# MechaCritter/Python-Visual-Similarity

Hardware: AMD Instinct MI355X
Metric: images/sec encoded + top-k retrieved, VLAD K256 RootSIFT (higher is better)
Workload: dtype f32

## Files before the change

### include/pvsim.h

```cpp
#ifndef PVSIM_H
#define PVSIM_H

#include <stddef.h>
#include <stdint.h>

#ifdef __cplusplus
extern "C" {
#endif

#define PVS_VERSION 103

typedef enum {
  PVS_OK = 0,
  PVS_ERR_INVALID = 1,
  PVS_ERR_NO_DEVICE = 2,
  PVS_ERR_OOM = 3,
  PVS_ERR_UNSUPPORTED = 4,
  PVS_ERR_DIM = 5,
  PVS_ERR_CAPACITY = 6
} pvs_status;

typedef enum {
  PVS_DESC_F32 = 0,
  PVS_DESC_F32_ROOTSIFT = 1,
  PVS_DESC_U8_ROOTSIFT = 2
} pvs_desc_kind;

typedef enum {
  PVS_OPT_ASSIGN_PREFILTER = 0,
  PVS_OPT_VLAD_PATH = 1,
  PVS_OPT_TOPK_SELECT_ONLY = 2,
  PVS_OPT_AGG_VARIANT = 3,
  PVS_OPT_FISHER_SCALE = 4,
  PVS_OPT_TRAIN_BATCH_CHUNKS = 5,
  PVS_OPT_UPDATE_WINDOW_ROWS = 6,
  PVS_OPT_SQ8_PATH = 7,
  PVS_OPT_COUNT_ = 8
} pvs_option;

typedef struct pvs_ctx pvs_ctx;
typedef struct pvs_codebook pvs_codebook;
typedef struct pvs_gmm pvs_gmm;
typedef struct pvs_pca pvs_pca;
typedef struct pvs_comm pvs_comm;

typedef struct {
  double power_norm_weight;
  double norm_order;
  double epsilon;
} pvs_norm_params;

int pvs_version(void);
const char* pvs_last_error(void);
int pvs_device_count(int* count);
int pvs_init(int device_id, void* stream, pvs_ctx** out);
int pvs_destroy(pvs_ctx* ctx);
int pvs_sync(pvs_ctx* ctx);
void* pvs_stream(pvs_ctx* ctx);
int pvs_device_name(pvs_ctx* ctx, char* buf, size_t buflen);
int pvs_set_option(pvs_ctx* ctx, int option, int value);
// ... 292 lines not shown
```

### include/pvsim_diag.h

```cpp
#ifndef PVSIM_DIAG_H
#define PVSIM_DIAG_H

#include "pvsim.h"

#ifdef __cplusplus
extern "C" {
#endif

int pvs_fused_profile(pvs_ctx* ctx, int enable, int64_t* out16);

#ifdef __cplusplus
}
#endif
#endif
```

### python-visual-similarity_amd/csrc/api.hip

```cpp
#include <algorithm>
#include <cmath>
#include <limits>
#include <memory>

#include "panel_plan.hpp"

namespace pvs {

static thread_local char g_err[512] = "";

void set_error(const char* fmt, ...) {
  va_list ap;
  va_start(ap, fmt);
  vsnprintf(g_err, sizeof(g_err), fmt, ap);
  va_end(ap);
}

static_assert(WS_UPDATE + 1 == pvs_ctx::NWS, "one block per WsSlot");

int ws_reserve(pvs_ctx* ctx, WsSlot which, size_t bytes, void** out) {
  if (bytes == 0) bytes = 16;
  if (ctx->ws_bytes[which] < bytes) {
    if (ctx->ws[which]) {
      PVS_HIP(hipStreamSynchronize(ctx->stream));
// ... 142 lines not shown
  return PVS_OK;
}

PVS_EXPORT int pvs_destroy(pvs_ctx* ctx) {
  if (!ctx) return PVS_OK;
  hipSetDevice(ctx->device);
  hipStreamSynchronize(ctx->stream);
  drain_timers(ctx);
  for (hipEvent_t e : ctx->event_pool) (void)hipEventDestroy(e);
  ctx->event_pool.clear();
  for (auto& kv : ctx->block_cache) (void)hipFree(kv.second);
  ctx->block_cache.clear();
  if (ctx->h_stage) (void)hipHostFree(ctx->h_stage);
  for (int i = 0; i < pvs_ctx::DSIFT_RING; ++i) {
    if (ctx->dsift_h[i]) (void)hipHostFree(ctx->dsift_h[i]);
    if (ctx->dsift_ev[i]) (void)hipEventDestroy(ctx->dsift_ev[i]);
  }
  for (int i = 0; i < pvs_ctx::NWS; ++i)
    if (ctx->ws[i]) hipFree(ctx->ws[i]);
  for (auto& p : ctx->gemm_plan)
    if (p.d_tiles) hipFree(p.d_tiles);
  if (ctx->d_queue) hipFree(ctx->d_queue);
  if (ctx->d_fused_stamps) hipFree(ctx->d_fused_stamps);
  if (ctx->owns_stream) hipStreamDestroy(ctx->stream);
  delete ctx;
  return PVS_OK;
}

PVS_EXPORT int pvs_sync(pvs_ctx* ctx) {
  PVS_NEED(ctx, "ctx");
  PVS_HIP(hipStreamSynchronize(ctx->stream));
  return PVS_OK;
}

PVS_EXPORT void* pvs_stream(pvs_ctx* ctx) { return ctx ? static_cast<void*>(ctx->stream) : nullptr; }

PVS_EXPORT int pvs_device_name(pvs_ctx* ctx, char* buf, size_t buflen) {
  PVS_NEED(ctx, "ctx");
  PVS_NEED(buf, "buf");
  hipDeviceProp_t prop;
  PVS_HIP(hipGetDeviceProperties(&prop, ctx->device));
  snprintf(buf, buflen, "%s (%s, %d CUs)", prop.name, prop.gcnArchName, prop.multiProcessorCount);
  return PVS_OK;
}

PVS_EXPORT int pvs_set_option(pvs_ctx* ctx, int option, int value) {
// ... 978 lines not shown
  PVS_HIP(hipMemcpyAsync(h_indices, d_indices, (size_t)n_clusters * 8, hipMemcpyDeviceToHost, ctx->stream));
  PVS_HIP(hipStreamSynchronize(ctx->stream));
  return PVS_OK;
}

PVS_EXPORT int pvs_fused_profile(pvs_ctx* ctx, int enable, int64_t* out16) {
  PVS_NEED(ctx, "ctx");
  PVS_HIP(hipSetDevice(ctx->device));
  PVS_HIP(hipStreamSynchronize(ctx->stream));
  if (out16) {
    for (int i = 0; i < 16; ++i) out16[i] = 0;
    if (ctx->d_fused_stamps) PVS_HIP(hipMemcpy(out16, ctx->d_fused_stamps, 16 * 8, hipMemcpyDeviceToHost));
  }
  if (enable) {
    if (!ctx->d_fused_stamps) PVS_HIP(hipMalloc(reinterpret_cast<void**>(&ctx->d_fused_stamps), 16 * 8));
    PVS_HIP(hipMemset(ctx->d_fused_stamps, 0, 16 * 8));
  } else if (ctx->d_fused_stamps) {
    PVS_HIP(hipFree(ctx->d_fused_stamps));
    ctx->d_fused_stamps = nullptr;
  }
  return PVS_OK;
}

PVS_EXPORT int pvs_timers_enable(pvs_ctx* ctx, int on) {
  PVS_NEED(ctx, "ctx");
  PVS_TRY(drain_timers(ctx));
  ctx->timers_on = on != 0;
  return PVS_OK;
}
PVS_EXPORT int pvs_timers_reset(pvs_ctx* ctx) {
  PVS_NEED(ctx, "ctx");
  PVS_TRY(drain_timers(ctx));
  for (int i = 0; i < PVS_TIMER_SLOTS; ++i) {
    ctx->t_total[i] = 0;
    ctx->t_count[i] = 0;
  }
  return PVS_OK;
}
PVS_EXPORT int pvs_timers_read(pvs_ctx* ctx, int which, double* total_ms, int64_t* launches) {
  PVS_NEED(ctx, "ctx");
  if (which < 0 || which >= PVS_TIMER_SLOTS) PVS_FAIL(PVS_ERR_INVALID, "timer slot %d out of range", which);
  PVS_TRY(drain_timers(ctx));
  if (total_ms) *total_ms = ctx->t_total[which];
  if (launches) *launches = ctx->t_count[which];
  return PVS_OK;
}
// ... 1 lines not shown
```

### python-visual-similarity_amd/csrc/assign_prefilter.hpp

```cpp
#pragma once

#include "common.hpp"
#include "desc_load.hpp"

namespace pvs {

typedef _Float16 f16x8_t __attribute__((ext_vector_type(8)));
typedef _Float16 f16x4_t __attribute__((ext_vector_type(4)));

constexpr int ASSIGN_THREADS = 512;
constexpr int ASSIGN_ROWS = (ASSIGN_THREADS / 64) * 32;

struct Assign16Args {
  const void* X;
  int64_t total;
  int D, ld;
  const _Float16* C16;
  const float* cnorm;
  int K_pad, D_pad16;
  int c_shift;
  float cmax;
  const _Float16* cnk;
  int cn_e1, K;
  int32_t* labels;
  int64_t* amb_rows;
  unsigned long long* amb_count;
  int64_t cap;
  float2* rowstat;
  unsigned long long* stamps;
  int nprod;
  int shape16;
};

int launch_assign16x(pvs_ctx* ctx, const Assign16Args& p, int kind, size_t lds, int grid);

__device__ __forceinline__ void pf_fill_sqrt_table(uint32_t* lds_t) {
  if (threadIdx.x < 256) {
    const float sv = sqrtf((float)threadIdx.x);
    const _Float16 hi = (_Float16)sv, lo = (_Float16)(sv - (float)hi);
    lds_t[threadIdx.x] = (uint32_t)__builtin_bit_cast(unsigned short, hi) | ((uint32_t)__builtin_bit_cast(unsigned short, lo) << 16);
  }
}
__device__ __forceinline__ void pf_u8_fragment(const uint32_t* lds_t, const uint32_t* xw, f16x8_t* xh, f16x8_t* xl) {
  uint32_t hw[4], lw[4];
#pragma unroll
  for (int i = 0; i < 2; ++i)
#pragma unroll
    for (int pq = 0; pq < 2; ++pq) {
      const uint32_t w = xw[i];
      const uint32_t e0 = lds_t[(w >> (16 * pq)) & 0xffu], e1 = lds_t[(w >> (16 * pq + 8)) & 0xffu];
      hw[2 * i + pq] = __builtin_amdgcn_perm(e1, e0, 0x05040100u);
      lw[2 * i + pq] = __builtin_amdgcn_perm(e1, e0, 0x07060302u);
    }
  *xh = __builtin_bit_cast(f16x8_t, make_uint4(hw[0], hw[1], hw[2], hw[3]));
  *xl = __builtin_bit_cast(f16x8_t, make_uint4(lw[0], lw[1], lw[2], lw[3]));
}

// ... 26 lines not shown
```

### python-visual-similarity_amd/csrc/common.hpp

```cpp
#pragma once
#include <hip/hip_runtime.h>

#include <cmath>
#include <cstdarg>
#include <cstdint>
#include <cstdio>
#include <cstring>
#include <map>
#include <type_traits>
#include <vector>

#include "../../include/pvsim.h"
#include "../../include/pvsim_diag.h"
#include "workspace.hpp"

#define PVS_EXPORT extern "C" __attribute__((visibility("default")))

namespace pvs {

void set_error(const char* fmt, ...);

#define PVS_FAIL(code, ...)        \
  do {                             \
    ::pvs::set_error(__VA_ARGS__); \
// ... 27 lines not shown

struct TimerRec {
  hipEvent_t a, b;
  int slot;
};

}

struct pvs_ctx {
  int device = 0;
  hipStream_t stream = nullptr;
  bool owns_stream = false;
  int num_cu = 256;
  static constexpr int NWS = 18;
  void* ws[NWS] = {};
  size_t ws_bytes[NWS] = {};
  struct GemmPlanSlot {
    int key[4] = {-1, -1, -1, -1};
    int n_main = 0, n_tail = 0, splitk = 1;
    void* d_tiles = nullptr;
    size_t cap = 0;
  } gemm_plan[5];
  std::map<const void*, int> lds_attr;
  int opt[PVS_OPT_COUNT_] = {1, 0, 0, 0, 0, 0, 0, 0};
  unsigned int* d_queue = nullptr;
  unsigned long long* d_fused_stamps = nullptr;
  bool timers_on = false;
  std::vector<pvs::TimerRec> pending;
  std::vector<hipEvent_t> event_pool;
  std::multimap<size_t, void*> block_cache;
  std::map<void*, size_t> block_size;
  size_t block_cache_bytes = 0;
  void* h_stage = nullptr;
  size_t h_stage_bytes = 0;
  static constexpr int DSIFT_RING = 4;
  void* dsift_h[DSIFT_RING] = {};
  size_t dsift_h_bytes[DSIFT_RING] = {};
  hipEvent_t dsift_ev[DSIFT_RING] = {};
  int dsift_next = 0;
  double t_total[PVS_TIMER_SLOTS] = {0};
  int64_t t_count[PVS_TIMER_SLOTS] = {0};
};

struct pvs_codebook {
  int K = 0, D = 0;
  int K_pad = 0, D_pad = 0;
  float* d_cent = nullptr;
  float* d_cpad = nullptr;
  float* d_cnorm = nullptr;
// ... 169 lines not shown
```

### python-visual-similarity_amd/csrc/vlad.hip

```cpp
#include "assign_prefilter.hpp"

namespace pvs {

typedef float f32x16 __attribute__((ext_vector_type(16)));

struct AssignArgs {
  const void* X;
  int64_t total;
  int D, ld;
  const float* Cpad;
  const float* cnorm;
  int K_pad, D_pad;
  int32_t* labels;
  const int64_t* rows;
  const unsigned long long* nrows;
  int64_t rows_cap;
};

constexpr int ASSIGN_DCHUNK = 128;

template <int NT, int KIND, bool VEC>
__global__ __launch_bounds__(ASSIGN_THREADS, 2) void assign_kernel(AssignArgs a) {
  extern __shared__ __attribute__((aligned(16))) char smem[];
  constexpr int CB = 32 * NT;
// ... 2 lines not shown
  float* lds_c = reinterpret_cast<float*>(smem);
  float* lds_n = lds_c + CB * stride;

  const int lane = threadIdx.x & 63, wave = threadIdx.x >> 6;
  const int j = lane & 31, h = lane >> 5;
  const int ncb = a.K_pad / CB;
  const int nsc = (a.D_pad + ASSIGN_DCHUNK - 1) / ASSIGN_DCHUNK;
  const bool restage = (ncb * nsc) > 1;
  const int64_t n_items = a.rows ? (int64_t)a.nrows[blockIdx.x] : a.total;
  const int64_t nblocks = (n_items + ASSIGN_ROWS - 1) / ASSIGN_ROWS;
  const int64_t* const my_rows = a.rows ? a.rows + (int64_t)blockIdx.x * a.rows_cap : nullptr;

  auto stage = [&](int cb, int sc) {
    const int cw = min(ASSIGN_DCHUNK, a.D_pad - sc * ASSIGN_DCHUNK);
    const int c4n = cw >> 2;
    for (int idx = threadIdx.x; idx < CB * c4n; idx += ASSIGN_THREADS) {
      const int r = idx / c4n, c4 = idx - r * c4n;
      const float4 v = *reinterpret_cast<const float4*>(a.Cpad + (int64_t)(cb * CB + r) * a.D_pad +
                                                        sc * ASSIGN_DCHUNK + 4 * c4);
      *reinterpret_cast<float4*>(lds_c + r * stride + 4 * c4) = v;
    }
    for (int idx = threadIdx.x; idx < CB; idx += ASSIGN_THREADS) lds_n[idx] = a.cnorm[cb * CB + idx];
  };

  if (!restage) {
    stage(0, 0);
    __syncthreads();
  }

  for (int64_t blk = my_rows ? 0 : blockIdx.x; blk < nblocks; blk += my_rows ? 1 : gridDim.x) {
    const int64_t item = blk * ASSIGN_ROWS + wave * 32 + j;
    const bool rvalid = item < n_items;
    const int64_t row = (my_rows && rvalid) ? my_rows[item] : item;
    float best = INFINITY;
    int bidx = 0;

    for (int cb = 0; cb < ncb; ++cb) {
      f32x16 acc[NT];
#pragma unroll
      for (int t = 0; t < NT; ++t)
#pragma unroll
        for (int r = 0; r < 16; ++r) acc[t][r] = 0.f;

      for (int sc = 0; sc < nsc; ++sc) {
        if (restage) {
          __syncthreads();
// ... 485 lines not shown
  if (total <= 0) return PVS_OK;
  const bool rs = kind != PVS_DESC_F32;
  if (rs && cb->D > ASSIGN_DCHUNK)
    PVS_FAIL(PVS_ERR_UNSUPPORTED, "fused RootSIFT needs D <= %d (got %d)", ASSIGN_DCHUNK, cb->D);
  const int nt = assign_tiles_for(cb->K);
  if (cb->K_pad % (32 * nt) != 0) PVS_FAIL(PVS_ERR_INVALID, "codebook padding does not match the tile count");
  AssignArgs a{d_desc, total, cb->D, ld, cb->d_cpad, cb->d_cnorm, cb->K_pad, cb->D_pad, d_labels, nullptr, nullptr, 0};
  const int esz = kind == PVS_DESC_U8_ROOTSIFT ? 1 : 4;
  const bool vec = (cb->D % 4 == 0) && (ld % 4 == 0) && ((reinterpret_cast<uintptr_t>(d_desc) % (4 * esz)) == 0);
  const int cw = cb->D_pad < ASSIGN_DCHUNK ? cb->D_pad : ASSIGN_DCHUNK;
  const size_t lds = (size_t)(32 * nt) * (cw + 4) * 4 + (size_t)(32 * nt) * 4;
  const int64_t nblocks = (total + ASSIGN_ROWS - 1) / ASSIGN_ROWS;
  const int grid = (int)(nblocks < ctx->num_cu ? nblocks : ctx->num_cu);
  ScopedTimer tm(ctx, T_ASSIGN);
  const bool pre = cb->d_c16 != nullptr && total >= 4096 && ctx->opt[PVS_OPT_ASSIGN_PREFILTER] != 0;
  if (pre) {
    const int64_t cap = (nblocks + grid - 1) / grid * ASSIGN_ROWS;
    char* ws = nullptr;
    const bool stat = rowstat_out != nullptr && kind == PVS_DESC_U8_ROOTSIFT;
    WsLayout<> lay;
    const auto cnt_p = lay.add<unsigned long long>((size_t)grid);
    const auto rows_p = lay.add<int64_t>((size_t)grid * cap);
    const auto stat_p = lay.add<float2>(stat ? (size_t)total : 0);
    PVS_TRY(ws_reserve(ctx, WS_LISTS, lay.bytes(), &ws));
    unsigned long long* cnt = cnt_p(ws);
    int64_t* rows = rows_p(ws);
    float2* rowstat = stat ? stat_p(ws) : nullptr;
    if (stat) *rowstat_out = rowstat;
    Assign16Args p{d_desc, total, cb->D, ld, static_cast<const _Float16*>(cb->d_c16), cb->d_cnorm, cb->K_pad, cb->D_pad16,
                   cb->c16_shift, cb->cmax, static_cast<const _Float16*>(cb->d_cnk), cb->cn_e1, cb->K, d_labels, rows, cnt, cap, rowstat,
                   ctx->d_fused_stamps, ctx->opt[PVS_OPT_ASSIGN_PREFILTER] == 2 ? 2 : (ctx->opt[PVS_OPT_ASSIGN_PREFILTER] == 3 ? 1 : 3),
                   ctx->opt[PVS_OPT_ASSIGN_PREFILTER] == 4 ? 1 : 0};
    const size_t lds16 = (size_t)2 * cb->K_pad * (128 + 8) * 2 + (size_t)cb->K_pad * 4 + (size_t)cb->K_pad * 8 + 1024;
    PVS_TRY(launch_assign16(ctx, p, kind, cb->K_pad / 32, vec, lds16, grid));
    a.rows = rows;
    a.nrows = cnt;
    a.rows_cap = cap;
  }
  return dispatch_desc_kind(kind, [&](auto k) { return launch_assign_kind<decltype(k)::value>(ctx, a, nt, vec, lds, grid); });
}

struct AggArgs {
  const void* X;
  int D, ld;
  const int64_t* offsets;
  const int32_t* labels;
  const float* cent;
  int K;
  float power, eps;
  int norm_mode;
  float norm_p;
  float* out;
  float* inv_norm;
  const float2* rowstat;
};

constexpr int AGG_THREADS = 256;
constexpr int AGG_WAVES = AGG_THREADS / 64;
constexpr int AGG_CHUNK = 4096;

// ... 497 lines not shown
```

### python-visual-similarity_amd/csrc/vlad_fused.hip

```cpp
#include "common.hpp"
#include "desc_load.hpp"

namespace pvs {

typedef float f32x16 __attribute__((ext_vector_type(16)));
typedef _Float16 f16x8_t __attribute__((ext_vector_type(8)));
typedef _Float16 f16x4_t __attribute__((ext_vector_type(4)));

constexpr int FU_THREADS = 512;
constexpr int FU_R = 64;
constexpr int FU_XS = 132;
constexpr int FU_TS = 1056;
constexpr int FU_TILE = 8 * FU_TS;
constexpr int FU_UNUSABLE = 0x7fffffff;
constexpr int FU_KB = 4;

constexpr int FU_OFF_X32 = 0;
constexpr int FU_OFF_XH = FU_OFF_X32 + FU_R * FU_XS * 4;
constexpr int FU_OFF_XL = FU_OFF_XH + 2 * FU_TILE;
constexpr int FU_OFF_NX = FU_OFF_XL + 2 * FU_TILE;
constexpr int FU_OFF_XSH = FU_OFF_NX + 256;
constexpr int FU_OFF_CAND = FU_OFF_XSH + 256;
constexpr int FU_OFF_ENT = FU_OFF_CAND + 8 * FU_R * 8;
constexpr int FU_OFF_ENTV = FU_OFF_ENT + 2048;
constexpr int FU_OFF_ROWSQ = FU_OFF_ENTV + 4096;
constexpr int FU_OFF_MISC = FU_OFF_ROWSQ + 1024;
constexpr int FU_LDS = FU_OFF_MISC + 64;

struct FusedArgs {
  const void* X;
// ... 294 lines not shown
          if (wave == 0 && ne > 0) {
            int e = ebase;
            for (int w = 0; w < 8; ++w)
              if (cm & (1 << w)) {
                const int sidx = 31 - (__float_as_int(s_cand[w * FU_R + lane].x) & 31);
                s_ent[e++] = lane | (w << 8) | (((am >> w) & 1) << 12) | (sidx << 16);
              }
          }
          __syncthreads();
          for (int e0 = 0; e0 < E; e0 += 16) {
            const int e = e0 + 2 * wave + h;
            const bool elive = e < E;
            const int ent = elive ? s_ent[e] : 0;
            const int er = ent & 0xff, ew = (ent >> 8) & 7, eall = (ent >> 12) & 1, esi = (ent >> 16) & 31;
            const int k = 32 * ew + (eall ? j : esi);
            const bool active = elive && (eall || j == 0);
            const float* xr = x32 + er * FU_XS;
            const float* cr = a.cpad + (size_t)k * 128;
            float dot = 0.f;
#pragma unroll 2
            for (int b8 = 0; b8 < 128; b8 += 8) {
              const float4 xa = *reinterpret_cast<const float4*>(xr + b8), xb = *reinterpret_cast<const float4*>(xr + b8 + 4);
              const float4 ca = *reinterpret_cast<const float4*>(cr + b8), cb = *reinterpret_cast<const float4*>(cr + b8 + 4);
              dot = fmaf(ca.x, xa.x, dot); dot = fmaf(cb.x, xb.x, dot);
              dot = fmaf(ca.y, xa.y, dot); dot = fmaf(cb.y, xb.y, dot);
              dot = fmaf(ca.z, xa.z, dot); dot = fmaf(cb.z, xb.z, dot);
              dot = fmaf(ca.w, xa.w, dot); dot = fmaf(cb.w, xb.w, dot);
            }
            const float v = fmaf(-2.f, dot, a.cnorm[k]);
            const bool ok = active && (v < INFINITY);
            float vv = ok ? v : INFINITY;
            int kk = ok ? k : 0x7fffffff;
#pragma unroll
            for (int m = 16; m >= 1; m >>= 1) {
              const float ov = __shfl_xor(vv, m, 64);
              const int okk = __shfl_xor(kk, m, 64);
              const bool take = ov < vv || (ov == vv && okk < kk);
              vv = take ? ov : vv;
              kk = take ? okk : kk;
            }
            if (elive && j == 0) s_entv[e] = make_float2(vv, __int_as_float(kk));
          }
          __syncthreads();
          if (rvalid && !settled) {
            float bv = INFINITY;
            int bk = 0x7fffffff;
            for (int i = 0; i < ne; ++i) {
              const float2 r = s_entv[ebase + i];
              const int rk = __float_as_int(r.y);
              if (r.x < bv || (r.x == bv && rk < bk)) { bv = r.x; bk = rk; }
// ... 154 lines not shown
```

### python-visual-similarity_amd/pvsim/_ffi.py

```python
from __future__ import annotations

import ctypes as C
import os
import threading

import numpy as np

from ._errors import CapacityError

_HERE = os.path.dirname(os.path.abspath(__file__))
LIB_PATH = os.environ.get("PVSIM_LIB", os.path.join(_HERE, "libpvsim_hip.so"))

PVS_OK, PVS_ERR_INVALID, PVS_ERR_NO_DEVICE, PVS_ERR_OOM, PVS_ERR_UNSUPPORTED, PVS_ERR_DIM, PVS_ERR_CAPACITY = range(7)
_EXC = {PVS_ERR_INVALID: ValueError, PVS_ERR_NO_DEVICE: RuntimeError, PVS_ERR_OOM: MemoryError,
        PVS_ERR_UNSUPPORTED: NotImplementedError, PVS_ERR_DIM: RuntimeError, PVS_ERR_CAPACITY: CapacityError}

DESC_F32, DESC_F32_ROOTSIFT, DESC_U8_ROOTSIFT = 0, 1, 2
OPT_ASSIGN_PREFILTER, OPT_VLAD_PATH, OPT_TOPK_SELECT_ONLY, OPT_AGG_VARIANT, OPT_FISHER_SCALE = 0, 1, 2, 3, 4
OPT_TRAIN_BATCH_CHUNKS = 5
PIX_U8_RGB, PIX_U8_GRAY, PIX_F32_RGB, PIX_F32_GRAY = 0, 1, 2, 3
DSIFT_U8, DSIFT_F32, DSIFT_F32_RAW, DSIFT_F32_QUANT = 0, 1, 2, 3
OPT_UPDATE_WINDOW_ROWS = 6
OPT_SQ8_PATH = 7
SQ8_PATH_AUTO, SQ8_PATH_ROWS, SQ8_PATH_MATRIX = 0, 1, 2
SQ8_MAX_L = 131072
RANGE_UPPER = 1
RANGE_PATH_AUTO, RANGE_PATH_EXACT, RANGE_PATH_FILTERED = 0, 1, 2
RANGE_MAX_CAPACITY = 1 << 40
SUBSET_PATH_AUTO, SUBSET_PATH_MASK, SUBSET_PATH_LISTED = 0, 1, 2
SUBSET_MAX_K = 1024
SCAN_TILE = 2048
COMBINE_CHUNK_BYTES, COMBINE_BATCH = 8192, 8
DIFFUSE_DOT_BLOCK, DIFFUSE_MAX_COLUMNS = 256, 65536
KRR_MAX_K1, KRR_MAX_KQ = 64, 1024
VLAD_PATH_AUTO, VLAD_PATH_GATHER, VLAD_PATH_STREAM, VLAD_PATH_FUSED = 0, 1, 2, 3
TIMER_NAMES = ("assign", "aggregate", "cosine_gemm", "topk", "fisher_posterior", "fisher_moments", "misc", "rescore")


class NormParams(C.Structure):
    _fields_ = [("power_norm_weight", C.c_double), ("norm_order", C.c_double), ("epsilon", C.c_double)]


_vp, _i64, _int, _sz = C.c_void_p, C.c_int64, C.c_int, C.c_size_t
_pp = C.POINTER(C.c_void_p)
_np = C.POINTER(NormParams)

# ... 111 lines not shown
    "pvs_krr_members_dev": [_vp, _vp, _vp, _vp, _i64, _int, _vp, _vp],
    "pvs_krr_weights_dev": [_vp, _vp, _vp, _i64, _int, _int, _vp, _vp],
    "pvs_krr_expand_dev": [_vp, _vp, _vp, _vp, _i64, _int, _int, _vp, _vp, _vp],
    "pvs_krr_query_dev": [_vp, _vp, _vp, _vp, _vp, _vp, _i64, _int, _int, _int, _int, _vp, _vp, _i64, _int, _vp, _vp, _vp, _vp],
    "pvs_krr_score_dev": [_vp, _vp, _vp, _vp, _vp, _i64, _int, _vp, _vp, _vp, _vp, _i64, _int, _int, C.c_double, _vp],
    "pvs_asmk_aggregate_dev": [_vp, _vp, _vp, _int, _vp, _vp, _i64, _i64, _vp, _vp, _int, _vp, _vp, _vp],
    "pvs_asmk_aggregate_ma_dev": [_vp, _vp, _vp, _int, _vp, _vp, _i64, _i64, _vp, _int, _vp, _int, _vp, _vp, _vp],
    "pvs_asmk_score_dev": [_vp, _i64, _vp, _vp, _vp, _int, _int, _vp, _vp, _vp, _i64, _vp, _vp, _vp, _vp, _int, _vp, _i64],
    "pvs_asmk_invert_dev": [_vp, _int, _int, _vp, _vp, _i64, _vp, _vp, _vp, _i64, _int, _vp, _vp, _vp],
    "pvs_asmk_weight_sums_dev": [_vp, _int, _vp, _vp, _i64, _vp, _vp, _vp, _vp],
    "pvs_asmk_insert_dev": [_vp, _int, _int, _vp, _vp, _vp, _vp, _vp, _vp, _vp, _vp, _vp, _vp, _vp],
    "pvs_asmk_remove_dev": [_vp, _int, _int, _i64, _vp, _vp, _vp, _vp, _vp, _vp, _vp, _vp, _vp],
    "pvs_asmk_expand_dev": [_vp, _i64, _vp, _vp, _vp, _int, _int, _vp, _vp, _vp, _i64, _int, _vp, _vp, _int, _int, _int, _vp, _int, _int,
                            _vp, _vp, _vp, _vp],
    "pvs_sq8_encode_dev": [_vp, _vp, _i64, _int, _vp, _vp],
    "pvs_sq8_topk_dev": [_vp, _vp, _vp, _i64, _vp, _vp, _i64, _int, _int, _i64, _int, _vp, _vp],
    "pvs_cosine_range_dev": [_vp, _vp, _i64, _vp, _i64, _i64, _vp, _vp, C.c_float, _int, _int, _int, _i64, _vp, _vp, _vp, _vp, _vp],
    "pvs_pair_components_dev": [_vp, _vp, _vp, _i64, _i64, _vp, _vp],
    "pvs_subset_create": [_vp, _vp, _i64, _i64, _pp],
    "pvs_subset_destroy": [_vp, _vp],
    "pvs_cosine_topk_subset_dev": [_vp, _vp, _i64, _vp, _i64, _i64, _vp, _vp, _vp, _int, _int, _int, _vp, _vp, _vp],
    "pvs_sq8_topk_subset_dev": [_vp, _vp, _vp, _i64, _vp, _vp, _i64, _int, _vp, _int, _int, _int, _vp, _vp, _vp],
    "pvs_fused_profile": [_vp, _int, _vp],
    "pvs_timers_enable": [_vp, _int],
    "pvs_timers_reset": [_vp],
    "pvs_timers_read": [_vp, _int, C.POINTER(C.c_double), C.POINTER(C.c_int64)],
}

_lib = None
_lock = threading.Lock()


def mapped_hip_runtimes() -> list[str]:
    found = []
    try:
        with open("/proc/self/maps") as f:
            for line in f:
                path = line.rsplit(None, 1)[-1] if "/" in line else ""
                if "libamdhip64" in os.path.basename(path) and path not in found:
                    found.append(path)
    except OSError:
        pass
    return found


def _one_hip_runtime() -> None:
# ... 56 lines not shown
```

### python-visual-similarity_amd/pvsim/engine.py

```python
from __future__ import annotations

import ctypes as C
import os
import sys
import threading

import numpy as np

from . import _ffi
from ._ffi import DESC_F32, DESC_F32_ROOTSIFT, DESC_U8_ROOTSIFT, check, norm_params, ptr

__all__ = ["Context", "default_context", "pack_descriptors", "dsift_count", "dsift_frames", "sift_workspace", "diffuse_workspace", "DESC_F32", "DESC_F32_ROOTSIFT", "DESC_U8_ROOTSIFT"]


def pack_descriptors(desc_list, dim: int, dtype=np.float32):
    counts = [0 if d is None else int(d.shape[0]) for d in desc_list]
    offsets = np.zeros(len(desc_list) + 1, dtype=np.int64)
    np.cumsum(counts, out=offsets[1:])
    packed = np.empty((int(offsets[-1]), dim), dtype=dtype)
    for d, o in zip(desc_list, offsets[:-1]):
        if d is not None and d.shape[0]:
            if d.shape[1] != dim:
                raise RuntimeError(f"descriptor dimension {d.shape[1]} does not match the model input dimension {dim}")
            packed[o:o + d.shape[0]] = d
# ... 824 lines not shown
        bs = np.empty((total_desc + 4095) // 4096, dtype=np.float64)
        check(_ffi.lib().pvs_min_update_dev(self.handle, ptr(d_mind), ptr(d_dist), total_desc, ptr(bs)))
        return bs

    def kmeanspp_run_dev(self, d_x, D, total_desc, n_clusters, trials, uniform, first_index):
        u = np.ascontiguousarray(uniform, dtype=np.float64).reshape(-1)
        if u.size < max(n_clusters - 1, 0) * trials:
            raise ValueError("need (n_clusters - 1) x trials uniform numbers")
        idx = np.full(n_clusters, -1, dtype=np.int64)
        idx[0] = first_index
        if u.size == 0:
            u = np.zeros(1)
        check(_ffi.lib().pvs_kmeanspp_run_dev(self.handle, ptr(d_x), D, total_desc, n_clusters, trials, ptr(u), ptr(idx)))
        return idx

    def fused_profile(self, enable=True, raw=False):
        out = np.zeros(16, dtype=np.int64)
        check(_ffi.lib().pvs_fused_profile(self.handle, int(enable), ptr(out)))
        if raw:
            return out
        names = ("P0", "A", "reduce", "reevaluate", "K2", "epilogue", "image_switch", "_", "stages", "stages_reevaluated", "entries", "rows_unsettled")
        return {n: int(v) for n, v in zip(names, out) if n != "_"}

    def timers_enable(self, on=True):
        check(_ffi.lib().pvs_timers_enable(self.handle, int(on)))

    def timers_reset(self):
        check(_ffi.lib().pvs_timers_reset(self.handle))

    def timers(self) -> dict:
        out = {}
        for i, name in enumerate(_ffi.TIMER_NAMES):
            ms, cnt = C.c_double(), C.c_int64()
            check(_ffi.lib().pvs_timers_read(self.handle, i, C.byref(ms), C.byref(cnt)))
            out[name] = (ms.value, cnt.value)
        return out


_default = None
_default_lock = threading.Lock()


def default_context() -> Context:
    global _default
    if _default is None or _default.handle is None:
        with _default_lock:
# ... 4 lines not shown
```

Baseline: 418,600.

## Add near-candidate exact resolution pass for ambiguous assignment rows

Adds a kernel that takes the rows the fp16 prefilter left ambiguous and recomputes their distances to all 256 centroids with split-precision MFMA. It then collects the few centroids within an error bound and checks them with exact fp32 dot products. Only rows with too many candidates or unusable numerics go on to the full exact assignment kernel. The aim is to shrink the expensive full reassignment workload, at the cost of an extra launch and workspace. It is on by default when K=256 and D=128, and a diagnostic stats counter is added.

New measurement: 419,600 (median of 6 runs). About the same (+0.2%).

```diff
diff --git a/include/pvsim.h b/include/pvsim.h
--- a/include/pvsim.h
+++ b/include/pvsim.h
@@ -35,7 +35,8 @@
   PVS_OPT_TRAIN_BATCH_CHUNKS = 5,
   PVS_OPT_UPDATE_WINDOW_ROWS = 6,
   PVS_OPT_SQ8_PATH = 7,
-  PVS_OPT_COUNT_ = 8
+  PVS_OPT_ASSIGN_NEAR = 8,
+  PVS_OPT_COUNT_ = 9
 } pvs_option;
 
 typedef struct pvs_ctx pvs_ctx;
diff --git a/include/pvsim_diag.h b/include/pvsim_diag.h
--- a/include/pvsim_diag.h
+++ b/include/pvsim_diag.h
@@ -9,6 +9,8 @@
 
 int pvs_fused_profile(pvs_ctx* ctx, int enable, int64_t* out16);
 
+int pvs_assign_near_stats(pvs_ctx* ctx, int enable, int64_t* out3);
+
 #ifdef __cplusplus
 }
 #endif
diff --git a/python-visual-similarity_amd/csrc/api.hip b/python-visual-similarity_amd/csrc/api.hip
--- a/python-visual-similarity_amd/csrc/api.hip
+++ b/python-visual-similarity_amd/csrc/api.hip
@@ -188,6 +188,7 @@
     if (p.d_tiles) hipFree(p.d_tiles);
   if (ctx->d_queue) hipFree(ctx->d_queue);
   if (ctx->d_fused_stamps) hipFree(ctx->d_fused_stamps);
+  if (ctx->d_near_stats) hipFree(ctx->d_near_stats);
   if (ctx->owns_stream) hipStreamDestroy(ctx->stream);
   delete ctx;
   return PVS_OK;
@@ -1212,6 +1213,24 @@
   return PVS_OK;
 }
 
+PVS_EXPORT int pvs_assign_near_stats(pvs_ctx* ctx, int enable, int64_t* out3) {
+  PVS_NEED(ctx, "ctx");
+  PVS_HIP(hipSetDevice(ctx->device));
+  PVS_HIP(hipStreamSynchronize(ctx->stream));
+  if (out3) {
+    for (int i = 0; i < 3; ++i) out3[i] = 0;
+    if (ctx->d_near_stats) PVS_HIP(hipMemcpy(out3, ctx->d_near_stats, 3 * 8, hipMemcpyDeviceToHost));
+  }
+  if (enable) {
+    if (!ctx->d_near_stats) PVS_HIP(hipMalloc(reinterpret_cast<void**>(&ctx->d_near_stats), 4 * 8));
+    PVS_HIP(hipMemset(ctx->d_near_stats, 0, 4 * 8));
+  } else if (ctx->d_near_stats) {
+    PVS_HIP(hipFree(ctx->d_near_stats));
+    ctx->d_near_stats = nullptr;
+  }
+  return PVS_OK;
+}
+
 PVS_EXPORT int pvs_timers_enable(pvs_ctx* ctx, int on) {
   PVS_NEED(ctx, "ctx");
   PVS_TRY(drain_timers(ctx));
diff --git a/python-visual-similarity_amd/csrc/assign_near.hip b/python-visual-similarity_amd/csrc/assign_near.hip
--- /dev/null
+++ b/python-visual-similarity_amd/csrc/assign_near.hip
@@ -0,0 +1,317 @@
+#include "assign_prefilter.hpp"
+
+namespace pvs {
+
+typedef float f32x16 __attribute__((ext_vector_type(16)));
+
+template <int KIND>
+__global__ __launch_bounds__(ASSIGN_THREADS, 1) void assign_near_kernel(Assign16Args a, AssignNearArgs nr) {
+  extern __shared__ __attribute__((aligned(16))) char smem[];
+  __shared__ unsigned int s_fb;
+  constexpr int NT = 8, CB = 32 * NT;
+  constexpr int stride = 128 + 8;
+  constexpr bool LUT = KIND == PVS_DESC_U8_ROOTSIFT;
+  _Float16* lds_h = reinterpret_cast<_Float16*>(smem);
+  _Float16* lds_l = lds_h + CB * stride;
+  _Float16* lds_k = lds_l + CB * stride;
+  uint32_t* lds_t = reinterpret_cast<uint32_t*>(lds_k + 4 * CB);
+  const int lane = threadIdx.x & 63, wave = threadIdx.x >> 6;
+  const int j = lane & 31, h = lane >> 5;
+
+  const int64_t n_items = (int64_t)a.amb_count[blockIdx.x];
+  if (n_items == 0) {
+    if (threadIdx.x == 0) nr.fb_count[blockIdx.x] = 0ull;
+    return;
+  }
+  const int64_t* const my_rows = a.amb_rows + (int64_t)blockIdx.x * a.cap;
+  int64_t* const fb_rows = nr.fb_rows + (int64_t)blockIdx.x * a.cap;
+
+  for (int idx = threadIdx.x; idx < 2 * CB * 16; idx += ASSIGN_THREADS) {
+    const int r = idx >> 4, c8 = idx & 15;
+    *reinterpret_cast<uint4*>(lds_h + r * stride + 8 * c8) = *reinterpret_cast<const uint4*>(a.C16 + (int64_t)r * 128 + 8 * c8);
+  }
+  for (int idx = threadIdx.x; idx < CB; idx += ASSIGN_THREADS)
+    *reinterpret_cast<uint2*>(lds_k + 4 * idx) = *reinterpret_cast<const uint2*>(a.cnk + 4 * idx);
+  if constexpr (LUT) pf_fill_sqrt_table(lds_t);
+  if (threadIdx.x == 0) s_fb = 0u;
+  __syncthreads();
+  const float sqrt_d = sqrtf((float)a.D);
+  unsigned int st_cand = 0, st_fb = 0, st_pairs = 0;
+
+  const int64_t nblocks = (n_items + ASSIGN_ROWS - 1) / ASSIGN_ROWS;
+  for (int64_t blk = 0; blk < nblocks; ++blk) {
+    const int64_t item = blk * ASSIGN_ROWS + wave * 32 + j;
+    const bool rvalid = item < n_items;
+    const int64_t row = my_rows[rvalid ? item : 0];
+
+    float xf[8][8];
+    uint32_t xw[8][2];
+    if constexpr (LUT) {
+      const uint8_t* pr = static_cast<const uint8_t*>(a.X) + row * a.ld + 4 * h;
+#pragma unroll
+      for (int t = 0; t < 8; ++t) {
+        xw[t][0] = *reinterpret_cast<const uint32_t*>(pr + 16 * t);
+        xw[t][1] = *reinterpret_cast<const uint32_t*>(pr + 16 * t + 8);
+      }
+    } else {
+#pragma unroll
+      for (int t = 0; t < 8; ++t) {
+        const float4 v0 = load4<KIND>(a.X, row, a.ld, 16 * t + 4 * h);
+        const float4 v1 = load4<KIND>(a.X, row, a.ld, 16 * t + 4 * h + 8);
+        xf[t][0] = v0.x; xf[t][1] = v0.y; xf[t][2] = v0.z; xf[t][3] = v0.w;
+        xf[t][4] = v1.x; xf[t][5] = v1.y; xf[t][6] = v1.z; xf[t][7] = v1.w;
+      }
+    }
+    float nx;
+    int x_shift = 0;
+    bool finite;
+    f16x8_t xh[8], xl[8];
+    _Float16 lut_f1 = (_Float16)0.f, lut_f2 = (_Float16)0.f;
+    float lut_sd = 1.f;
+    if constexpr (LUT) {
+      unsigned ssum = 0;
+#pragma unroll
+      for (int t = 0; t < 8; ++t) {
+        ssum = __builtin_amdgcn_sad_u8(xw[t][0], 0u, ssum);
+        ssum = __builtin_amdgcn_sad_u8(xw[t][1], 0u, ssum);
+      }
+      ssum += __shfl_xor(ssum, 32, 64);
+      const float sf = (float)ssum, dd = sf + 1e-7f;
+      lut_sd = sqrtf(dd);
+      const float ff = ldexpf(lut_sd, a.cn_e1);
+      lut_f1 = (_Float16)ff;
+      lut_f2 = (_Float16)(ff - (float)lut_f1);
+      finite = ff >= 0.125f && ff <= 32768.f;
+      nx = sqrtf(sf) * 1.0001f;
+#pragma unroll
+      for (int t = 0; t < 8; ++t) pf_u8_fragment(lds_t, xw[t], &xh[t], &xl[t]);
+    } else {
+      float n2 = 0.f, amax = 0.f, rs_r = 0.f;
+      if constexpr (DescTraits<KIND>::rootsift) {
+        float s = 0.f, rmax = 0.f;
+#pragma unroll
+        for (int t = 0; t < 8; ++t)
+#pragma unroll
+          for (int q = 0; q < 8; ++q) {
+            s += xf[t][q];
+            rmax = fmaxf(rmax, xf[t][q]);
+          }
+        s += __shfl_xor(s, 32, 64);
+        rmax = fmaxf(rmax, __shfl_xor(rmax, 32, 64));
+        rs_r = 1.0f / (s + 1e-7f);
+        n2 = s * rs_r * 1.0001f;
+        amax = __builtin_amdgcn_sqrtf(rmax * rs_r) * 1.0001f;
+        if (!(s >= 0.f) || !(rmax * rs_r <= 3.0e38f)) n2 = NAN;
+      } else {
+#pragma unroll
+        for (int t = 0; t < 8; ++t)
+#pragma unroll
+          for (int q = 0; q < 8; ++q) {
+            n2 = fmaf(xf[t][q], xf[t][q], n2);
+            amax = fmaxf(amax, fabsf(xf[t][q]));
+          }
+        n2 += __shfl_xor(n2, 32, 64);
+        amax = fmaxf(amax, __shfl_xor(amax, 32, 64));
+      }
+      nx = sqrtf(n2) * 1.0001f;
+      int ex = 13;
+      if (amax > 0.f) (void)frexpf(amax, &ex);
+      x_shift = 13 - ex;
+      finite = nx <= 3.0e38f;
+      if (x_shift > 40 || x_shift < -40) { finite = false; x_shift = 0; }
+      if (x_shift + a.cn_e1 < -14 || x_shift + a.cn_e1 > 15) finite = false;
+      const float xs = ldexpf(1.f, x_shift);
+      const float rs_rs = rs_r * xs * xs;
+#pragma unroll
+      for (int t = 0; t < 8; ++t)
+#pragma unroll
+        for (int q = 0; q < 8; ++q) {
+          float v;
+          if constexpr (DescTraits<KIND>::rootsift) v = __builtin_amdgcn_sqrtf(xf[t][q] * rs_rs);
+          else v = xf[t][q] * xs;
+          const _Float16 hi = (_Float16)v;
+          xh[t][q] = hi;
+          xl[t][q] = (_Float16)(v - (float)hi);
+        }
+    }
+    const float m2s = -2.f * ldexpf(1.f, -(x_shift + a.c_shift));
+    __builtin_amdgcn_sched_barrier(0);
+
+    f16x8_t cnb;
+    {
+      const _Float16 pw = (h == 0 && finite) ? (_Float16)ldexpf(1.f, x_shift + a.cn_e1) : (_Float16)0.f;
+#pragma unroll
+      for (int q = 0; q < 8; ++q) cnb[q] = (_Float16)0.f;
+      if constexpr (LUT) {
+        if (h == 0 && finite) { cnb[0] = lut_f1; cnb[1] = lut_f2; cnb[2] = lut_f1; cnb[3] = lut_f2; cnb[4] = lut_f1; cnb[5] = lut_f2; }
+      } else {
+        cnb[0] = pw; cnb[1] = pw; cnb[2] = pw;
+      }
+    }
+    f32x16 acc[NT];
+    const f32x16 zero16 = {0.f, 0.f, 0.f, 0.f, 0.f, 0.f, 0.f, 0.f, 0.f, 0.f, 0.f, 0.f, 0.f, 0.f, 0.f, 0.f};
+#pragma unroll
+    for (int g = 0; g < NT / 2; ++g) {
+#pragma unroll
+      for (int t = 0; t < 8; ++t) {
+        f16x8_t fh[2], fl[2];
+#pragma unroll
+        for (int u = 0; u < 2; ++u) {
+          fh[u] = *reinterpret_cast<const f16x8_t*>(lds_h + (32 * (2 * g + u) + j) * stride + 16 * t + 8 * h);
+          fl[u] = *reinterpret_cast<const f16x8_t*>(lds_l + (32 * (2 * g + u) + j) * stride + 16 * t + 8 * h);
+        }
+#pragma unroll
+        for (int u = 0; u < 2; ++u) acc[2 * g + u] = __builtin_amdgcn_mfma_f32_32x32x16_f16(fl[u], xh[t], t == 0 ? zero16 : acc[2 * g + u], 0, 0, 0);
+#pragma unroll
+        for (int u = 0; u < 2; ++u) acc[2 * g + u] = __builtin_amdgcn_mfma_f32_32x32x16_f16(fh[u], xl[t], acc[2 * g + u], 0, 0, 0);
+#pragma unroll
+        for (int u = 0; u < 2; ++u) acc[2 * g + u] = __builtin_amdgcn_mfma_f32_32x32x16_f16(fh[u], xh[t], acc[2 * g + u], 0, 0, 0);
+        __builtin_amdgcn_sched_barrier(0);
+      }
+#pragma unroll
+      for (int u = 0; u < 2; ++u) {
+        const f16x4_t pk = *reinterpret_cast<const f16x4_t*>(lds_k + 4 * (32 * (2 * g + u) + j));
+        f16x8_t ca;
+#pragma unroll
+        for (int q = 0; q < 8; ++q) ca[q] = (_Float16)0.f;
+        if constexpr (LUT) {
+          if (h == 0) { ca[0] = pk[0]; ca[1] = pk[0]; ca[2] = pk[1]; ca[3] = pk[1]; ca[4] = pk[2]; ca[5] = pk[2]; }
+        } else {
+          if (h == 0) { ca[0] = pk[0]; ca[1] = pk[1]; ca[2] = pk[2]; }
+        }
+        acc[2 * g + u] = __builtin_amdgcn_mfma_f32_32x32x16_f16(ca, cnb, acc[2 * g + u], 0, 0, 0);
+      }
+    }
+
+    float smax = -INFINITY, chk = 0.f;
+#pragma unroll
+    for (int tile = 0; tile < NT; ++tile)
+#pragma unroll
+      for (int r = 0; r < 16; ++r) {
+        smax = fmaxf(smax, acc[tile][r]);
+        chk = fmaf(acc[tile][r], 0.f, chk);
+      }
+    smax = fmaxf(smax, __shfl_xor(smax, 32, 64));
+    chk += __shfl_xor(chk, 32, 64);
+    const float best = smax * m2s;
+    const float eps = prefilter_eps<KIND, 3, LUT>(nx, a.cmax, lut_sd, sqrt_d);
+    const float thr = best + 2.f * eps;
+    uint32_t mask[NT / 2] = {0u, 0u, 0u, 0u};
+#pragma unroll
+    for (int tile = 0; tile < NT; ++tile)
+#pragma unroll
+      for (int r = 0; r < 16; ++r)
+        mask[tile >> 1] |= (acc[tile][r] * m2s <= thr ? 1u : 0u) << (16 * (tile & 1) + r);
+    int ncand = __popc(mask[0]) + __popc(mask[1]) + __popc(mask[2]) + __popc(mask[3]);
+    ncand += __shfl_xor(ncand, 32, 64);
+    bool padded = false;
+    if (a.K < CB) {
+#pragma unroll
+      for (int tile = 0; tile < NT; ++tile)
+#pragma unroll
+        for (int r = 0; r < 16; ++r)
+          if (32 * tile + (r & 3) + 8 * (r >> 2) + 4 * h >= a.K && ((mask[tile >> 1] >> (16 * (tile & 1) + r)) & 1u)) padded = true;
+    }
+    padded = __shfl_xor((int)padded, 32, 64) != 0 || padded;
+    const bool usable = finite && chk == 0.f && fabsf(best) <= 3.0e38f && !padded && ncand >= 1 && ncand <= NEAR_SLOTS;
+    if (!usable || !rvalid) { mask[0] = 0u; mask[1] = 0u; mask[2] = 0u; mask[3] = 0u; }
+
+    __builtin_amdgcn_sched_barrier(0);
+    float bv = INFINITY;
+    int bk = 0x7fffffff;
+    if (__ballot((mask[0] | mask[1] | mask[2] | mask[3]) != 0u) != 0ull) {
+      float xr[128];
+      if constexpr (KIND == PVS_DESC_U8_ROOTSIFT) {
+        uint32_t w[32];
+        unsigned ssum = 0;
+#pragma unroll
+        for (int q = 0; q < 32; ++q) {
+          w[q] = *reinterpret_cast<const uint32_t*>(static_cast<const uint8_t*>(a.X) + row * a.ld + 4 * q);
+          ssum = __builtin_amdgcn_sad_u8(w[q], 0u, ssum);
+        }
+        const RootsiftRow<KIND> rr((float)ssum);
+#pragma unroll
+        for (int q = 0; q < 32; ++q) {
+          xr[4 * q + 0] = rr(float(w[q] & 0xffu));
+          xr[4 * q + 1] = rr(float((w[q] >> 8) & 0xffu));
+          xr[4 * q + 2] = rr(float((w[q] >> 16) & 0xffu));
+          xr[4 * q + 3] = rr(float(w[q] >> 24));
+        }
+      } else {
+#pragma unroll
+        for (int q = 0; q < 32; ++q) {
+          const float4 v = load4<KIND>(a.X, row, a.ld, 4 * q);
+          xr[4 * q + 0] = v.x; xr[4 * q + 1] = v.y; xr[4 * q + 2] = v.z; xr[4 * q + 3] = v.w;
+        }
+        if constexpr (DescTraits<KIND>::rootsift) {
+          float sh[2] = {0.f, 0.f};
+#pragma unroll
+          for (int t = 0; t < 16; ++t)
+#pragma unroll
+            for (int hh = 0; hh < 2; ++hh) sh[hh] += (xr[8 * t + 4 * hh] + xr[8 * t + 4 * hh + 1]) + (xr[8 * t + 4 * hh + 2] + xr[8 * t + 4 * hh + 3]);
+          const RootsiftRow<KIND> rr(sh[0] + sh[1]);
+#pragma unroll
+          for (int i = 0; i < 128; ++i) xr[i] = rr(xr[i]);
+        }
+      }
+      for (;;) {
+        const uint32_t any = mask[0] | mask[1] | mask[2] | mask[3];
+        if (__ballot(any != 0u) == 0ull) break;
+        if (any != 0u) {
+          const int mi = mask[0] ? 0 : (mask[1] ? 1 : (mask[2] ? 2 : 3));
+          const uint32_t m = mi == 0 ? mask[0] : (mi == 1 ? mask[1] : (mi == 2 ? mask[2] : mask[3]));
+          const int bit = __ffs(m) - 1;
+          const uint32_t cleared = m & (m - 1u);
+          if (mi == 0) mask[0] = cleared; else if (mi == 1) mask[1] = cleared; else if (mi == 2) mask[2] = cleared; else mask[3] = cleared;
+          const int tile = 2 * mi + (bit >> 4), r = bit & 15;
+          const int k = 32 * tile + (r & 3) + 8 * (r >> 2) + 4 * h;
+          const float* cr = nr.cpad + (size_t)k * 128;
+          float dot = 0.f;
+#pragma unroll
+          for (int part = 0; part < 4; ++part) {
+            float4 c4[8];
+#pragma unroll
+            for (int q = 0; q < 8; ++q) c4[q] = *reinterpret_cast<const float4*>(cr + 32 * part + 4 * q);
+#pragma unroll
+            for (int q = 0; q < 4; ++q) {
+              const int b8 = 32 * part + 8 * q;
+              dot = assign_exact_dot8(dot, make_float4(xr[b8], xr[b8 + 1], xr[b8 + 2], xr[b8 + 3]),
+                                      make_float4(xr[b8 + 4], xr[b8 + 5], xr[b8 + 6], xr[b8 + 7]), c4[2 * q], c4[2 * q + 1]);
+            }
+          }
+          const float v = fmaf(-2.f, dot, a.cnorm[k]);
+          if (v < INFINITY && (v < bv || (v == bv && k < bk))) { bv = v; bk = k; }
+          ++st_pairs;
+        }
+      }
+    }
+    {
+      const float ov = __shfl_xor(bv, 32, 64);
+      const int ok = __shfl_xor(bk, 32, 64);
+      if (ov < bv || (ov == bv && ok < bk)) { bv = ov; bk = ok; }
+    }
+    const int label = bv < INFINITY ? bk : 0;
+    const bool leader = h == 0 && rvalid;
+    st_cand += (unsigned)__popcll(__ballot(leader && usable));
+    st_fb += (unsigned)__popcll(__ballot(leader && !usable));
+    pf_label_or_list(a, usable, leader, row, label, lane, &s_fb, fb_rows);
+  }
+  __syncthreads();
+  if (threadIdx.x == 0) nr.fb_count[blockIdx.x] = (unsigned long long)s_fb;
+  if (nr.stats != nullptr) {
+    for (int m = 32; m >= 1; m >>= 1) st_pairs += __shfl_xor(st_pairs, m, 64);
+    if (lane == 0) {
+      atomicAdd(nr.stats + 0, (unsigned long long)st_cand);
+      atomicAdd(nr.stats + 1, (unsigned long long)st_fb);
+      atomicAdd(nr.stats + 2, (unsigned long long)st_pairs);
+    }
+  }
+}
+
+int launch_assign_near(pvs_ctx* ctx, const Assign16Args& p, const AssignNearArgs& nr, int kind, size_t lds, int grid) {
+  return dispatch_desc_kind(kind, [&](auto k) {
+    return launch_lds(ctx, assign_near_kernel<decltype(k)::value>, dim3(grid), dim3(ASSIGN_THREADS), lds, p, nr);
+  });
+}
+
+}
diff --git a/python-visual-similarity_amd/csrc/assign_prefilter.hpp b/python-visual-similarity_amd/csrc/assign_prefilter.hpp
--- a/python-visual-similarity_amd/csrc/assign_prefilter.hpp
+++ b/python-visual-similarity_amd/csrc/assign_prefilter.hpp
@@ -33,6 +33,23 @@
 };
 
 int launch_assign16x(pvs_ctx* ctx, const Assign16Args& p, int kind, size_t lds, int grid);
+
+constexpr int NEAR_SLOTS = 8;
+struct AssignNearArgs {
+  const float* cpad;
+  int64_t* fb_rows;
+  unsigned long long* fb_count;
+  unsigned long long* stats;
+};
+int launch_assign_near(pvs_ctx* ctx, const Assign16Args& p, const AssignNearArgs& nr, int kind, size_t lds, int grid);
+
+__device__ __forceinline__ float assign_exact_dot8(float dot, const float4& xa, const float4& xb, const float4& ca, const float4& cb) {
+  dot = fmaf(ca.x, xa.x, dot); dot = fmaf(cb.x, xb.x, dot);
+  dot = fmaf(ca.y, xa.y, dot); dot = fmaf(cb.y, xb.y, dot);
+  dot = fmaf(ca.z, xa.z, dot); dot = fmaf(cb.z, xb.z, dot);
+  dot = fmaf(ca.w, xa.w, dot); dot = fmaf(cb.w, xb.w, dot);
+  return dot;
+}
 
 __device__ __forceinline__ void pf_fill_sqrt_table(uint32_t* lds_t) {
   if (threadIdx.x < 256) {
diff --git a/python-visual-similarity_amd/csrc/common.hpp b/python-visual-similarity_amd/csrc/common.hpp
--- a/python-visual-similarity_amd/csrc/common.hpp
+++ b/python-visual-similarity_amd/csrc/common.hpp
@@ -73,9 +73,10 @@
     size_t cap = 0;
   } gemm_plan[5];
   std::map<const void*, int> lds_attr;
-  int opt[PVS_OPT_COUNT_] = {1, 0, 0, 0, 0, 0, 0, 0};
+  int opt[PVS_OPT_COUNT_] = {1, 0, 0, 0, 0, 0, 0, 0, 0};
   unsigned int* d_queue = nullptr;
   unsigned long long* d_fused_stamps = nullptr;
+  unsigned long long* d_near_stats = nullptr;
   bool timers_on = false;
   std::vector<pvs::TimerRec> pending;
   std::vector<hipEvent_t> event_pool;
diff --git a/python-visual-similarity_amd/csrc/vlad.hip b/python-visual-similarity_amd/csrc/vlad.hip
--- a/python-visual-similarity_amd/csrc/vlad.hip
+++ b/python-visual-similarity_amd/csrc/vlad.hip
@@ -48,6 +48,8 @@
     }
     for (int idx = threadIdx.x; idx < CB; idx += ASSIGN_THREADS) lds_n[idx] = a.cnorm[cb * CB + idx];
   };
+
+  if (my_rows && n_items == 0) return;
 
   if (!restage) {
     stage(0, 0);
@@ -579,6 +581,11 @@
     const auto cnt_p = lay.add<unsigned long long>((size_t)grid);
     const auto rows_p = lay.add<int64_t>((size_t)grid * cap);
     const auto stat_p = lay.add<float2>(stat ? (size_t)total : 0);
+    const int pf_opt = ctx->opt[PVS_OPT_ASSIGN_PREFILTER];
+    const bool near = ctx->opt[PVS_OPT_ASSIGN_NEAR] == 0 && (pf_opt == 1 || pf_opt == 4) && vec && cb->D == 128 && cb->D_pad16 == 128 &&
+                      cb->D_pad == 128 && cb->K_pad == 256 && (reinterpret_cast<uintptr_t>(cb->d_cpad) % 16) == 0;
+    const auto fb_cnt_p = lay.add<unsigned long long>(near ? (size_t)grid : 0);
+    const auto fb_rows_p = lay.add<int64_t>(near ? (size_t)grid * cap : 0);
     PVS_TRY(ws_reserve(ctx, WS_LISTS, lay.bytes(), &ws));
     unsigned long long* cnt = cnt_p(ws);
     int64_t* rows = rows_p(ws);
@@ -593,6 +600,13 @@
     a.rows = rows;
     a.nrows = cnt;
     a.rows_cap = cap;
+    if (near) {
+      const AssignNearArgs nr{cb->d_cpad, fb_rows_p(ws), fb_cnt_p(ws), ctx->d_near_stats};
+      const size_t lds_near = (size_t)2 * 256 * (128 + 8) * 2 + (size_t)256 * 8 + 1024;
+      PVS_TRY(launch_assign_near(ctx, p, nr, kind, lds_near, grid));
+      a.rows = nr.fb_rows;
+      a.nrows = nr.fb_count;
+    }
   }
   return dispatch_desc_kind(kind, [&](auto k) { return launch_assign_kind<decltype(k)::value>(ctx, a, nt, vec, lds, grid); });
 }
diff --git a/python-visual-similarity_amd/csrc/vlad_fused.hip b/python-visual-similarity_amd/csrc/vlad_fused.hip
--- a/python-visual-similarity_amd/csrc/vlad_fused.hip
+++ b/python-visual-similarity_amd/csrc/vlad_fused.hip
@@ -1,11 +1,8 @@
-#include "common.hpp"
-#include "desc_load.hpp"
+#include "assign_prefilter.hpp"
 
 namespace pvs {
 
 typedef float f32x16 __attribute__((ext_vector_type(16)));
-typedef _Float16 f16x8_t __attribute__((ext_vector_type(8)));
-typedef _Float16 f16x4_t __attribute__((ext_vector_type(4)));
 
 constexpr int FU_THREADS = 512;
 constexpr int FU_R = 64;
@@ -346,10 +343,7 @@
             for (int b8 = 0; b8 < 128; b8 += 8) {
               const float4 xa = *reinterpret_cast<const float4*>(xr + b8), xb = *reinterpret_cast<const float4*>(xr + b8 + 4);
               const float4 ca = *reinterpret_cast<const float4*>(cr + b8), cb = *reinterpret_cast<const float4*>(cr + b8 + 4);
-              dot = fmaf(ca.x, xa.x, dot); dot = fmaf(cb.x, xb.x, dot);
-              dot = fmaf(ca.y, xa.y, dot); dot = fmaf(cb.y, xb.y, dot);
-              dot = fmaf(ca.z, xa.z, dot); dot = fmaf(cb.z, xb.z, dot);
-              dot = fmaf(ca.w, xa.w, dot); dot = fmaf(cb.w, xb.w, dot);
+              dot = assign_exact_dot8(dot, xa, xb, ca, cb);
             }
             const float v = fmaf(-2.f, dot, a.cnorm[k]);
             const bool ok = active && (v < INFINITY);
diff --git a/python-visual-similarity_amd/pvsim/_ffi.py b/python-visual-similarity_amd/pvsim/_ffi.py
--- a/python-visual-similarity_amd/pvsim/_ffi.py
+++ b/python-visual-similarity_amd/pvsim/_ffi.py
@@ -22,6 +22,7 @@
 DSIFT_U8, DSIFT_F32, DSIFT_F32_RAW, DSIFT_F32_QUANT = 0, 1, 2, 3
 OPT_UPDATE_WINDOW_ROWS = 6
 OPT_SQ8_PATH = 7
+OPT_ASSIGN_NEAR = 8
 SQ8_PATH_AUTO, SQ8_PATH_ROWS, SQ8_PATH_MATRIX = 0, 1, 2
 SQ8_MAX_L = 131072
 RANGE_UPPER = 1
@@ -179,6 +180,7 @@
     "pvs_cosine_topk_subset_dev": [_vp, _vp, _i64, _vp, _i64, _i64, _vp, _vp, _vp, _int, _int, _int, _vp, _vp, _vp],
     "pvs_sq8_topk_subset_dev": [_vp, _vp, _vp, _i64, _vp, _vp, _i64, _int, _vp, _int, _int, _int, _vp, _vp, _vp],
     "pvs_fused_profile": [_vp, _int, _vp],
+    "pvs_assign_near_stats": [_vp, _int, _vp],
     "pvs_timers_enable": [_vp, _int],
     "pvs_timers_reset": [_vp],
     "pvs_timers_read": [_vp, _int, C.POINTER(C.c_double), C.POINTER(C.c_int64)],
diff --git a/python-visual-similarity_amd/pvsim/engine.py b/python-visual-similarity_amd/pvsim/engine.py
--- a/python-visual-similarity_amd/pvsim/engine.py
+++ b/python-visual-similarity_amd/pvsim/engine.py
@@ -870,6 +870,11 @@
         names = ("P0", "A", "reduce", "reevaluate", "K2", "epilogue", "image_switch", "_", "stages", "stages_reevaluated", "entries", "rows_unsettled")
         return {n: int(v) for n, v in zip(names, out) if n != "_"}
 
+    def assign_near_stats(self, enable=True):
+        out = np.zeros(3, dtype=np.int64)
+        check(_ffi.lib().pvs_assign_near_stats(self.handle, int(enable), ptr(out)))
+        return {"rows_on_candidates": int(out[0]), "rows_passed_on": int(out[1]), "pairs": int(out[2])}
+
     def timers_enable(self, on=True):
         check(_ffi.lib().pvs_timers_enable(self.handle, int(on)))
 
```
